# kubeflow/Code-Intelligence

Hardware: NVIDIA H100
Metric: issues/sec to 2400-d @ seq_len 512 batch 256 (higher is better)
Workload: dtype bf16

## Files before the change

code_intelligence_b200/csrc/api.cu:

```cuda
#include <algorithm>
#include <cmath>
#include <cstdarg>
#include <cstdio>
#include <cstdlib>
#include <cstring>
#include <mutex>
#include <string>
#include <vector>

#include <cuda_fp16.h>

#include "../../include/issue_emb_b200.h"
#include "kernels.h"

namespace {

thread_local std::string g_last_error;

int fail(int code, const char* fmt, ...) {
  char buf[512];
  va_list ap;
  va_start(ap, fmt);
  vsnprintf(buf, sizeof(buf), fmt, ap);
  va_end(ap);
// ... 358 lines not shown
    CK(ie::launch_tokens_time_major(ids_dev, B, T, b_pad, c.vocab_sz, c.pad_idx, h->tok.as<int>(), h->err.as<int>(), s));
    h->launches++;
  }
  if (h->use_persistent) check_persistent(h, s);
  const bool persistent = h->use_persistent != 0;
  const size_t carry_layer = static_cast<size_t>(h->max_batch) * h->y_ld;
  CK(cudaMemsetAsync(h->hcarry.p, 0, static_cast<size_t>(c.n_layers) * carry_layer * sizeof(__nv_bfloat16), s));
  const size_t slot_bytes = static_cast<size_t>(b_pad) * h->y_ld * sizeof(__nv_bfloat16);

  for (long long t0 = 0; t0 < T; t0 += chunk_T) {
    const int Tc = static_cast<int>(std::min<long long>(chunk_T, T - t0));
    const long long crow = static_cast<long long>(Tc) * b_pad;
    if (!proj) {
      CK(ie::launch_embed_gather(ids_dev, B, T, b_pad, h->emb.as<__nv_bfloat16>(), c.vocab_sz, ring_mul * h->e_pad,
                                 h->x0.as<__nv_bfloat16>(), ring_mul * h->e_pad, c.pad_idx, h->err.as<int>(),
                                 static_cast<int>(t0), Tc, s));
      h->launches++;
    }
    if ((rc = mark(h, 1, s)) != IE_OK) return rc;
    int cur = 0;
    const __nv_bfloat16* layer_in = h->x0.as<__nv_bfloat16>();
    const __nv_bfloat16* prev_ring = nullptr;
    long long layer_in_ld = ring_mul * h->e_pad;
    for (int l = 0; l < c.n_layers; ++l) {
      const bool last = (l == c.n_layers - 1);
      Layer& L = h->layers[l];
      const bool from_table = proj && l == 0;
      const bool fused = persistent && last && l > 0 && h->segs == 1 && h->fuse_last && L.w_cat.p != nullptr;
      __nv_bfloat16* ybuf = h->y[cur].as<__nv_bfloat16>();
      __nv_bfloat16* carry = h->hcarry.as<__nv_bfloat16>() + static_cast<size_t>(l) * carry_layer;
      float* cstate = h->c.as<float>() + static_cast<size_t>(l) * h->max_batch * mop;
      CUtensorMap tm_h, tm_w;
      CK(ie::make_tmap_bf16_2d(&tm_h, ybuf, static_cast<uint64_t>(ring_mul) * L.kh_pad, static_cast<uint64_t>(crow + b_pad),
                               h->y_ld, 64, 128));
      if (fused)
        CK(ie::make_tmap_bf16_2d(&tm_w, L.w_cat.p, static_cast<uint64_t>(L.kin_pad + L.kh_pad), 4ull * L.out_pad,
                                 static_cast<uint64_t>(L.kin_pad + L.kh_pad), 64, 256));
      else
        CK(ie::make_tmap_bf16_2d(&tm_w, L.w_hh.p, static_cast<uint64_t>(ring_mul) * L.kh_pad, 4ull * L.out_pad,
                                 static_cast<uint64_t>(ring_mul) * L.kh_pad, 64, 256));
      CUtensorMap tm_h64 = tm_h;
      CUtensorMap tm_x = tm_h;
      if (fused)
        CK(ie::make_tmap_bf16_2d(&tm_x, prev_ring, static_cast<uint64_t>(L.kin_pad), static_cast<uint64_t>(crow + b_pad),
                                 h->y_ld, 64, 128));
      if (h->use_mc)
        CK(ie::make_tmap_bf16_2d(&tm_h64, ybuf, static_cast<uint64_t>(ring_mul) * L.kh_pad,
                                 static_cast<uint64_t>(crow + b_pad), h->y_ld, 64, 64));
      CK(cudaMemcpyAsync(ybuf, carry, slot_bytes, cudaMemcpyDeviceToDevice, s));
      if (!from_table && !fused) {
        ie::GemmArgs g{};
        fill_gemm(h, L, g);
        g.a = layer_in;
        g.lda = layer_in_ld;
        g.d = h->gx.p;
        g.m_pad = static_cast<int>(crow);
        g.m_store = static_cast<int>(crow);
        g.diag = h->diag.as<long long>() + 8 * l + 4;
        CK(ie::launch_gemm_bf16(g, s));
        h->launches++;
      }
      if ((rc = mark(h, 2 + 2 * l, s)) != IE_OK) return rc;

      if (persistent) CK(cudaMemsetAsync(h->step_done.p, 0, static_cast<size_t>(Tc) * ng * sizeof(unsigned), s));
      ie::LstmLayerArgs q{};
      q.tm_h = tm_h; q.tm_w = tm_w; q.tm_h64 = tm_h64; q.mc = h->use_mc; q.mc_ctas = h->mc_ctas;
      q.tm_x = tm_x; q.pre_nkb = fused ? L.kin_pad / 64 : 0; q.bias = L.bias.as<float>();
      q.gx = from_table ? h->proj.p : h->gx.p;
      q.tok = from_table ? h->tok.as<int>() : nullptr;
      q.c = cstate; q.y = ybuf;
      q.raw = (l == raw_layer && raw_out != nullptr) ? h->raw.as<float>() : nullptr;
      q.pool_sum = (last && pooled) ? h->pool_sum.as<float>() : nullptr;
      q.pool_max = h->pool_max.as<float>(); q.pool_last = h->pool_last.as<float>();
      q.lengths = h->lengths.as<int>();
      q.step_done = h->step_done.as<unsigned>();
      q.abort_flag = h->err.as<unsigned>() + 1; q.spin_limit = h->spin_limit;
      q.T = Tc; q.t0 = static_cast<int>(t0); q.T_total = T; q.ng = ng;
      q.u = L.u; q.n_cta = L.n_cta; q.out_pad = L.out_pad; q.kh_pad = L.kh_pad;
      q.ldy = h->y_ld; q.raw_ld = L.out_pad;
      q.gate_mode = h->gate_mode; q.gx_bf16 = h->gx_bf16; q.segs = h->segs;
      q.num_sms = h->num_sms; q.check_only = 0; q.cooperative = h->cooperative; q.fault = h->fault;
      q.diag = h->diag.as<long long>() + 8 * l;
      q.trace = nullptr;
      if (persistent) {
        if (l == h->trace_layer && t0 == 0) {
          const int ctas = ie::lstm_layer_ctas(q);
          const long long items = (static_cast<long long>(Tc) * ng * L.n_cta + ctas - 1) / ctas;
          CK(h->trace.reserve(static_cast<size_t>(ctas) * items * 12 * sizeof(long long), true));
          q.trace = h->trace.as<long long>();
          q.trace_items = static_cast<int>(items);
          h->trace_T = static_cast<int>(items);
          h->trace_ctas = ctas;
        }
        cudaError_t e = ie::launch_lstm_layer(q, s);
        if (e == cudaErrorCooperativeLaunchTooLarge) {
          cudaGetLastError();
          return fail(IE_ERR_STATE, "the persistent recurrent kernel cannot be co-resident on this device "
                                   "(cooperative launch refused); set IE_SEQ=0 for the per-timestep fallback");
        }
        CK(e);
// ... 826 lines not shown
```

code_intelligence_b200/csrc/gemm.cu:

```cuda
#include "gemm_kernel.cuh"

namespace ie {


cudaError_t launch_gemm_bf16(const GemmArgs& g, cudaStream_t stream) {
  if (g.m_pad % kBlockM || g.k_pad % kBlockK || g.bn % 16 || g.bn < 16 || g.bn > 256 || g.n_pad % g.bn ||
      g.n_store % 16 || g.ldd % 2)
    return cudaErrorInvalidValue;
  CUtensorMap tmA, tmB;
  const int segs = g.segs == 3 ? 3 : 1;
  const uint64_t k_inner = static_cast<uint64_t>(segs == 3 ? 2 : 1) * g.k_pad;
  const long long spin_limit = g.spin_limit > 0 ? g.spin_limit : kSpinLimitDefault;
  cudaError_t e = make_tmap_bf16_2d(&tmA, g.a, k_inner, g.m_pad, g.lda, kBlockK, kBlockM);
  if (e != cudaSuccess) return e;
  e = make_tmap_bf16_2d(&tmB, g.b, k_inner, g.n_pad, g.ldb, kBlockK, kBlockN);
  if (e != cudaSuccess) return e;

  const size_t smem = 1024 + static_cast<size_t>(kGemmStages) * kGemmStageBytes + 2 * kGemmStages * 8 + 32;
  const int num_m_blocks = g.m_pad / kBlockM;
  const int num_n_blocks = (g.n_pad + kBlockN - 1) / kBlockN;
  const int num_k_blocks = g.k_pad / kBlockK;
  const int num_tiles = num_m_blocks * num_n_blocks;
  const int sms = g.num_sms > 0 ? g.num_sms : 132;
  const int grid = num_tiles < sms ? num_tiles : sms;
  const int panel = 16;

#define IE_LAUNCH(OUT, ACT, FRAG)                                                                                  \
  do {                                                                                                             \
    auto kfn = gemm_bf16_kernel<OUT, ACT, FRAG>;                                                                       \
    e = cudaFuncSetAttribute(kfn, cudaFuncAttributeMaxDynamicSharedMemorySize, static_cast<int>(smem));            \
    if (e != cudaSuccess) return e;                                                                                \
    kfn<<<grid, kGemmThreads, smem, stream>>>(tmA, tmB, reinterpret_cast<OUT*>(g.d), g.bias, g.m_store, g.n_store, \
                                              g.ldd, num_m_blocks, num_n_blocks, num_k_blocks, panel, segs,        \
                                              g.k_pad, g.abort_flag, spin_limit, g.diag, DenseEpi{});              \
  } while (0)

  if (g.frag) {
    if (g.act != 0 || g.out_bf16 == 1 || g.bias == nullptr || g.n_store % kBlockN || g.n_store != g.n_pad ||
        (g.ldd * (g.out_bf16 == 2 ? 2 : 4)) % 16)
      return cudaErrorInvalidValue;
    if (g.out_bf16 == 2) IE_LAUNCH(__half, 0, true);
    else IE_LAUNCH(float, 0, true);
  } else if (g.out_bf16 == 2) {
    if (g.act != 0) return cudaErrorInvalidValue;
    IE_LAUNCH(__half, 0, false);
  } else if (g.out_bf16) {
    if (g.act == 0) IE_LAUNCH(__nv_bfloat16, 0, false);
    else if (g.act == 1) IE_LAUNCH(__nv_bfloat16, 1, false);
    else IE_LAUNCH(__nv_bfloat16, 2, false);
  } else {
    if (g.act == 0) IE_LAUNCH(float, 0, false);
// ... 9 lines not shown
```

code_intelligence_b200/csrc/gemm_kernel.cuh:

```cuda
#pragma once
#include <cuda_fp16.h>
#include <type_traits>

#include "kernels.h"
#include "ptx.cuh"

namespace ie {

struct DenseEpi {
  static constexpr bool kSliced = false;
  static constexpr uint64_t kHintA = kEvictNormal;
  static constexpr uint64_t kHintB = kEvictLast;
  struct State {};
};

namespace {

__device__ __forceinline__ uint32_t pack_f16x2(float lo, float hi) {
  const __half2 v = __floats2half2_rn(lo, hi);
  return *reinterpret_cast<const uint32_t*>(&v);
}

constexpr int kBlockM = 128;
constexpr int kBlockN = 256;
constexpr int kBlockK = 64;
constexpr int kGemmThreads = 384;
constexpr int kGemmStages = 4;
constexpr uint32_t kABytes = kBlockM * kBlockK * 2;
constexpr uint32_t kBBytes = kBlockN * kBlockK * 2;
constexpr uint32_t kGemmStageBytes = kABytes + kBBytes;

template <typename OutT, int ACT, bool FRAG, typename Epi = DenseEpi>
__global__ void __launch_bounds__(kGemmThreads, 1)
gemm_bf16_kernel(const __grid_constant__ CUtensorMap tmA, const __grid_constant__ CUtensorMap tmB, OutT* __restrict__ D,
                 const float* __restrict__ bias, int m_store, int n_store, long long ldd, int num_m_blocks,
                 int num_n_blocks, int num_k_blocks, int panel, int segs, int k_pad, unsigned* abort_flag,
                 long long spin_limit, long long* diag, const __grid_constant__ Epi epi) {
  extern __shared__ uint8_t smem_raw[];
  const uint32_t raw = smem_u32(smem_raw);
  uint8_t* smem = smem_raw + ((1024u - (raw & 1023u)) & 1023u);

  uint64_t* full_bar = reinterpret_cast<uint64_t*>(smem + kGemmStages * kGemmStageBytes);
  uint64_t* empty_bar = full_bar + kGemmStages;
  uint32_t* abort_s = reinterpret_cast<uint32_t*>(empty_bar + kGemmStages);
  const Abort ab{abort_s, abort_flag, spin_limit};
  const int nkt = num_k_blocks * segs;

  const int warp = threadIdx.x >> 5;
  const int lane = threadIdx.x & 31;

  if (warp == 0 && lane == 0) {
    tma_prefetch_desc(&tmA);
    tma_prefetch_desc(&tmB);
    if (diag != nullptr && blockIdx.x == 0) {
      unsigned long long g;
      asm volatile("mov.u64 %0, %%globaltimer;" : "=l"(g));
      diag[0] = clock64();
      diag[1] = static_cast<long long>(g);
    }
  }
  if (warp == 1 && lane == 0) {
    for (int s = 0; s < kGemmStages; ++s) {
      mbar_init(&full_bar[s], 1);
// ... 32 lines not shown
      uint32_t phase = 0;
      for (int tile = first_tile; tile < num_tiles && !aborted(ab); tile = next_tile(tile)) {
        int m_blk, n_blk;
        decode(tile, m_blk, n_blk);
        for (int kb = 0; kb < nkt; ++kb) {
          const int seg = kb / num_k_blocks, r = kb - seg * num_k_blocks;
          mbar_wait(&empty_bar[stage], phase ^ 1, ab);
          uint8_t* sa = smem + static_cast<size_t>(stage) * kGemmStageBytes;
          mbar_arrive_expect_tx(&full_bar[stage], kGemmStageBytes);
          tma_load_2d(sa, &tmA, &full_bar[stage], (seg == 1 ? k_pad : 0) + r * kBlockK, m_blk * kBlockM, Epi::kHintA);
          tma_load_2d(sa + kABytes, &tmB, &full_bar[stage], (seg == 2 ? k_pad : 0) + r * kBlockK, n_blk * kBlockN,
                      Epi::kHintB);
          if (++stage == kGemmStages) { stage = 0; phase ^= 1; }
        }
      }
    }
  } else {
    const int wg = (warp - 4) >> 2;
    const int q = lane & 3;
    const int rbase = wg * 64 + (warp & 3) * 16 + (lane >> 2);
    const uint32_t smem_base = smem_u32(smem);
    const bool signal = (threadIdx.x & 127) == 0;
    int stage = 0;
    uint32_t phase = 0;
    float d[128];
    typename Epi::State st{};
    for (int tile = first_tile; tile < num_tiles; tile = next_tile(tile)) {
      int m_blk, n_blk;
      decode(tile, m_blk, n_blk);
      int prev = -1;
      for (int kb = 0; kb < nkt; ++kb) {
        mbar_wait(&full_bar[stage], phase, ab);
        const uint32_t sa = smem_base + stage * kGemmStageBytes;
        const uint64_t da = wgmma_desc_sw128(sa + wg * (kABytes / 2));
        const uint64_t db = wgmma_desc_sw128(sa + kABytes);
        wgmma_fence();
#pragma unroll
        for (int k = 0; k < kBlockK / 16; ++k) wgmma_m64n256k16(d, da + 2 * k, db + 2 * k, (kb | k) != 0);
        wgmma_commit();
        if (prev >= 0) {
          wgmma_wait<1>();
          if (signal) mbar_arrive(&empty_bar[prev]);
        }
        prev = stage;
        if (++stage == kGemmStages) { stage = 0; phase ^= 1; }
      }
      wgmma_wait<0>();
      wgmma_fence_regs(d);
      if (signal && prev >= 0) mbar_arrive(&empty_bar[prev]);
      if constexpr (Epi::kSliced) {
        epi.tile(d, m_blk, n_blk, wg * 64 + (warp & 3) * 16, lane, st);
        continue;
      }
      if constexpr (FRAG) {
        constexpr int kPer = 16 / static_cast<int>(sizeof(OutT));
        const float4* bq = reinterpret_cast<const float4*>(bias) + n_blk * (kBlockN / 4) + q;
        OutT* drow[2];
#pragma unroll
        for (int hr = 0; hr < 2; ++hr)
          drow[hr] = D + static_cast<long long>(m_blk * kBlockM + rbase + 8 * hr) * ldd + n_blk * kBlockN + q * kPer;
#pragma unroll
        for (int k = 0; k < 64 / kPer; ++k) {
          float4 b[kPer / 4];
#pragma unroll
          for (int i = 0; i < kPer / 4; ++i) b[i] = __ldg(bq + 4 * (k * (kPer / 4) + i));
#pragma unroll
          for (int hr = 0; hr < 2; ++hr) {
            if (m_blk * kBlockM + rbase + 8 * hr >= m_store) continue;
// ... 64 lines not shown
```

code_intelligence_b200/csrc/kernels.h:

```cpp
#pragma once
#include <cuda.h>
#include <cuda_bf16.h>
#include <cuda_runtime.h>
#include <stddef.h>
#include <stdint.h>

namespace ie {

cudaError_t make_tmap_bf16_2d(CUtensorMap* out, const void* base, uint64_t inner, uint64_t rows, uint64_t ld,
                              uint32_t box_inner, uint32_t box_rows);

__host__ __device__ inline int frag_index(int c, int elem_bytes) {
  const int q = (c & 7) >> 1;
  const int ix = 4 * (c >> 4) + 2 * ((c >> 3) & 1) + (c & 1);
  const int per_chunk = 16 / elem_bytes;
  return (ix / per_chunk * 4 + q) * per_chunk + ix % per_chunk;
}

struct GemmArgs {
  const __nv_bfloat16* a;
  const __nv_bfloat16* b;
  void* d;
  const float* bias;
  int m_pad, n_pad, k_pad;
  long long lda, ldb, ldd;
  int m_store, n_store;
  int bn;
  int act;
  int out_bf16;
  int num_sms;
  int segs;
  unsigned* abort_flag;
  long long spin_limit;
  long long* diag;
  int frag;
};
cudaError_t launch_gemm_bf16(const GemmArgs& g, cudaStream_t stream);

constexpr int kMaxBatches = 12;
struct LstmLayerArgs {
// ... 80 lines not shown
```

code_intelligence_b200/csrc/knn.cu:

```cuda
#include <algorithm>

#include "gemm_kernel.cuh"

namespace ie {

namespace {

__device__ __forceinline__ uint32_t order_key(float s) {
  const uint32_t b = __float_as_uint(s);
  return (b & 0x80000000u) ? ~b : (b | 0x80000000u);
}
__device__ __forceinline__ float key_score(uint32_t k) {
  return __uint_as_float((k & 0x80000000u) ? (k & 0x7fffffffu) : ~k);
}

__device__ __noinline__ float knn_compact(uint2* buf, int count, int kp, int lane) {
  __syncwarp();
  uint32_t t = 0;
  for (int bit = 31; bit >= 0; --bit) {
    const uint32_t c = t | (1u << bit);
    int m = 0;
    for (int i = lane; i < count; i += 32) m += buf[i].x >= c;
    if (static_cast<int>(__reduce_add_sync(~0u, static_cast<unsigned>(m))) >= kp) t = c;
  }
// ... 376 lines not shown

void knn_plan(int nq, long long n, int kp, int num_sms, int* S, int* nbs) {
  const int m_blocks = (nq + 127) / 128;
  const long long n_blocks = (n + 255) / 256;
  long long s = std::max(1, num_sms / m_blocks);
  s = std::min<long long>(s, n_blocks);
  s = std::min<long long>(s, kKnnMergeMax / kp);
  *nbs = static_cast<int>((n_blocks + s - 1) / s);
  *S = static_cast<int>((n_blocks + *nbs - 1) / *nbs);
}

cudaError_t launch_knn_stage1(const KnnStage1Args& a, cudaStream_t stream) {
  if (a.m_pad % 128 || a.k_pad % 64 || a.nq > a.m_pad) return cudaErrorInvalidValue;
  CUtensorMap tmA, tmB;
  cudaError_t e = make_tmap_bf16_2d(&tmA, a.qs, 2ull * a.k_pad, a.m_pad, 2ull * a.k_pad, kBlockK, kBlockM);
  if (e != cudaSuccess) return e;
  e = make_tmap_bf16_2d(&tmB, a.xs, 2ull * a.k_pad, static_cast<uint64_t>(a.n), 2ull * a.k_pad, kBlockK, kBlockN);
  if (e != cudaSuccess) return e;
  KnnEpi epi{};
  epi.cand = a.cand;
  epi.cnt = a.cnt;
  epi.col = a.col;
  epi.rowt = a.rowt;
  epi.nq = a.nq;
  epi.n = static_cast<int>(a.n);
  epi.S = a.S;
  epi.nbs = a.nbs;
  epi.kp = a.kp;
  epi.cosine = a.cosine;
  epi.m_blocks = a.m_pad / kBlockM;
  epi.items = epi.m_blocks * a.S;
  const int num_n_blocks = static_cast<int>((a.n + kBlockN - 1) / kBlockN);
  const int grid = std::min(epi.items, a.num_sms > 0 ? a.num_sms : 132);
  const size_t smem = 1024 + static_cast<size_t>(kGemmStages) * kGemmStageBytes + 2 * kGemmStages * 8 + 32;
  auto kfn = gemm_bf16_kernel<float, 0, false, KnnEpi>;
  e = cudaFuncSetAttribute(kfn, cudaFuncAttributeMaxDynamicSharedMemorySize, static_cast<int>(smem));
  if (e != cudaSuccess) return e;
  kfn<<<grid, kGemmThreads, smem, stream>>>(tmA, tmB, nullptr, nullptr, 0, 0, 0, epi.m_blocks, num_n_blocks,
                                            a.k_pad / kBlockK, 16, 3, a.k_pad, nullptr, kSpinLimitDefault, nullptr, epi);
  return cudaGetLastError();
}

cudaError_t launch_knn_merge_rerank(const uint2* cand, const int* cnt, int rows, int S, int kp, const float* Q,
                                    const float* X, int D, int cosine, int k, float* out_dist, int64_t* out_idx,
                                    float* dbg_score, int64_t* dbg_idx, cudaStream_t stream) {
  int P = 1;
  while (P < S * kp) P <<= 1;
  const size_t smem = static_cast<size_t>(P) * 8 + static_cast<size_t>(kp) * 16;
  auto kfn = knn_merge_rerank_kernel;
  cudaError_t e = cudaFuncSetAttribute(kfn, cudaFuncAttributeMaxDynamicSharedMemorySize, static_cast<int>(smem));
  if (e != cudaSuccess) return e;
  kfn<<<rows, 512, smem, stream>>>(cand, cnt, S, kp, P, Q, X, D, cosine, k, out_dist, out_idx, dbg_score, dbg_idx);
  return cudaGetLastError();
}

}
```

code_intelligence_b200/csrc/lstm_layer.cu:

```cuda
#include <cmath>

#include <cuda_fp16.h>

#include "kernels.h"
#include "lstm_common.cuh"
#include "ptx.cuh"

namespace ie {

namespace {

constexpr int kLThreads = 384;
constexpr int kLStages = 4;
constexpr int kLTileN = 256;
constexpr int kLRows = 128;
constexpr uint32_t kHBytes = kLRows * 64 * 2;
constexpr uint32_t kWBytes = kLTileN * 64 * 2;
constexpr uint32_t kStageBytes = kHBytes + kWBytes;

__device__ __forceinline__ void st_release_cta(uint32_t* p, uint32_t v) {
  asm volatile("st.release.cta.shared::cta.u32 [%0], %1;" ::"r"(smem_u32(p)), "r"(v) : "memory");
}
__device__ __forceinline__ uint32_t ld_acquire_cta(const uint32_t* p) {
  uint32_t v;
  asm volatile("ld.acquire.cta.shared::cta.u32 %0, [%1];" : "=r"(v) : "r"(smem_u32(p)) : "memory");
  return v;
}
__device__ __forceinline__ void wait_seq_ge(const uint32_t* p, uint32_t target, const Abort& ab) {
  if (ld_acquire_cta(p) >= target) return;
  if (aborted(ab)) return;
  const long long t0 = clock64();
  uint32_t spins = 0;
  while (ld_acquire_cta(p) < target) {
    __nanosleep(64);
    if (((++spins) & 0x3Fu) == 0 && abort_poll(ab, t0)) return;
  }
}

struct KArgs {
  const void* gx;
  const int* tok;
  const float* bias;
  float* cstate;
  __nv_bfloat16* y;
  float* raw;
  float* pool_sum;
  float* pool_max;
  float* pool_last;
  const int* lengths;
  unsigned* step_done;
  unsigned* abort_flag;
  long long spin_limit;
  long long ldy, raw_ld;
  long long* trace;
  long long* diag;
  int T, t_begin, t0, T_total, ng, tiles, out_pad, nkb, segs, kh_pad, gate_mode, trace_items, fault;
  int pre_nkb;
};

template <bool TOK, bool GXBF, bool POOL, bool MC, bool FUSE>
__device__ __forceinline__ void lstm_layer_body(const CUtensorMap& tm_h, const CUtensorMap& tm_w,
                                                const CUtensorMap& tm_h64, const CUtensorMap& tm_x, const KArgs& a) {
  extern __shared__ uint8_t smem_raw[];
  const uint32_t rawaddr = smem_u32(smem_raw);
  uint8_t* smem = smem_raw + ((1024u - (rawaddr & 1023u)) & 1023u);

  uint8_t* ring = smem;
  uint64_t* full = reinterpret_cast<uint64_t*>(ring + kLStages * kStageBytes);
  uint64_t* empty = full + kLStages;
  uint32_t* cready = reinterpret_cast<uint32_t*>(empty + kLStages);
  uint32_t* abort_s = cready + 1;
  const Abort ab{abort_s, a.abort_flag, a.spin_limit};

  const int warp = threadIdx.x >> 5;
  const int lane = threadIdx.x & 31;
  long long* const trace = a.trace;
#define IE_TRACE(slot, kk) do { if (trace && (kk) < a.trace_items) { unsigned long long _g; \
    asm volatile("mov.u64 %0, %%globaltimer;" : "=l"(_g)); \
    trace[(static_cast<long long>(blockIdx.x) * a.trace_items + (kk)) * 12 + (slot)] = static_cast<long long>(_g); } } while (0)
  const uint32_t crank = MC ? cluster_ctarank() : 0u;
  const int P = static_cast<int>(gridDim.x);
  const int tiles = a.tiles, ng = a.ng;
  const int per_batch = 2 * tiles;
  const int C = ng * per_batch;
  const long long total = static_cast<long long>(a.T) * C;
  const int b_pad = 256 * ng;
  const int nkt = a.nkb * a.segs;
  const int pre = FUSE ? a.pre_nkb : 0;
  auto decode = [&](long long n, int& t, int& g, int& half, int& j) {
    const long long s = n / C;
    const int c = static_cast<int>(n - s * C);
    t = a.t_begin + static_cast<int>(s);
    g = c / per_batch;
    const int r = c - g * per_batch;
    half = r / tiles;
    j = r - half * tiles;
  };

  if (warp == 0 && lane == 0) {
    tma_prefetch_desc(&tm_h);
    tma_prefetch_desc(&tm_w);
    if (MC) tma_prefetch_desc(&tm_h64);
    if (FUSE) tma_prefetch_desc(&tm_x);
    if (a.diag != nullptr && blockIdx.x == 0) {
      unsigned long long g;
      asm volatile("mov.u64 %0, %%globaltimer;" : "=l"(g));
      a.diag[0] = clock64();
      a.diag[1] = static_cast<long long>(g);
    }
  }
  if (warp == 1 && lane == 0) {
    for (int s = 0; s < kLStages; ++s) {
      mbar_init(&full[s], 2);
      mbar_init(&empty[s], MC ? 4 : 2);
    }
    *cready = 0;
    *abort_s = 0;
    fence_barrier_init();
  }
  if (MC) cluster_sync();
  else __syncthreads();

  if (warp < 4) {
    if (warp == 0 && lane == 0) {
      int stage = 0;
      uint32_t phase = 0;
      int k = 0;
      for (long long n = blockIdx.x; n < total && !aborted(ab); n += P, ++k) {
        int t, g, half, j;
        decode(n, t, g, half, j);
        const int row0 = t * b_pad + g * 256 + half * kLRows;
        if constexpr (FUSE) {
          for (int kb = 0; kb < pre; ++kb) {
            mbar_wait(&empty[stage], phase ^ 1, ab);
            mbar_arrive_expect_tx(&full[stage], kHBytes);
            tma_load_2d(ring + stage * kStageBytes, &tm_x, &full[stage], kb * 64, row0 + b_pad, kEvictNormal);
            if (++stage == kLStages) { stage = 0; phase ^= 1; }
          }
        }
        wait_seq_ge(cready, static_cast<uint32_t>(k + 1), ab);
        if (t > a.t_begin) fence_proxy_async();
        IE_TRACE(0, k);
        for (int kb = 0; kb < nkt; ++kb) {
          mbar_wait(&empty[stage], phase ^ 1, ab);
          mbar_arrive_expect_tx(&full[stage], kHBytes);
          const int seg = kb / a.nkb, r = kb - seg * a.nkb;
          const int kc = (seg == 1 ? a.kh_pad : 0) + r * 64;
          if constexpr (MC) {
            tma_load_2d_mc(ring + stage * kStageBytes + crank * (kHBytes / 2), &tm_h64, &full[stage], kc,
                           row0 + static_cast<int>(crank) * (kLRows / 2), static_cast<uint16_t>(0x3), kEvictNormal);
          } else {
            tma_load_2d(ring + stage * kStageBytes, &tm_h, &full[stage], kc, row0, kEvictNormal);
          }
          if (++stage == kLStages) { stage = 0; phase ^= 1; }
        }
        IE_TRACE(1, k);
      }
    } else if (warp == 1 && lane == 0) {
      int stage = 0;
      uint32_t phase = 0;
      for (long long n = blockIdx.x; n < total && !aborted(ab); n += P) {
        int t, g, half, j;
        decode(n, t, g, half, j);
        for (int kb = 0; kb < pre + nkt; ++kb) {
          mbar_wait(&empty[stage], phase ^ 1, ab);
          mbar_arrive_expect_tx(&full[stage], kWBytes);
          const int seg = FUSE ? 0 : kb / a.nkb, r = kb - seg * a.nkb;
          tma_load_2d(ring + stage * kStageBytes + kHBytes, &tm_w, &full[stage], (seg == 2 ? a.kh_pad : 0) + r * 64,
                      j * kLTileN, kEvictLast);
          if (++stage == kLStages) { stage = 0; phase ^= 1; }
        }
      }
    } else if (warp == 2 && lane == 0) {
      int k = 0;
      for (long long n = blockIdx.x; n < total && !aborted(ab); n += P, ++k) {
        int t, g, half, j;
        decode(n, t, g, half, j);
        if (t > a.t_begin)
          wait_flag_ge_relaxed(a.step_done + (t - a.t_begin - 1) * ng + g, static_cast<unsigned>(per_batch), ab);
        st_release_cta(cready, static_cast<uint32_t>(k + 1));
      }
    }
  } else {
    const int wg = (warp - 4) >> 2;
    const int q = lane & 3;
    const int rbase = wg * 64 + (warp & 3) * 16 + (lane >> 2);
    const long long lo_off = a.segs > 1 ? a.kh_pad : 0;
    const uint32_t ring_base = smem_u32(ring);
    const bool signal = (threadIdx.x & 127) == 0;
    int stage = 0;
    uint32_t phase = 0;
    int k = 0;
    float d[128];
    for (long long n = blockIdx.x; n < total; n += P, ++k) {
      int t, g, half, j;
      decode(n, t, g, half, j);
      const int tg = a.t0 + t;
      int prev = -1;
      for (int kb = 0; kb < pre + nkt; ++kb) {
        mbar_wait(&full[stage], phase, ab);
        if (kb == pre && signal && wg == 0) IE_TRACE(2, k);
        const uint32_t sa = ring_base + stage * kStageBytes;
        const uint64_t da = wgmma_desc_sw128(sa + wg * (kHBytes / 2));
        const uint64_t db = wgmma_desc_sw128(sa + kHBytes);
        wgmma_fence();
#pragma unroll
        for (int kk = 0; kk < 4; ++kk) wgmma_m64n256k16(d, da + 2 * kk, db + 2 * kk, (kb | kk) != 0);
        wgmma_commit();
        if (prev >= 0) {
          wgmma_wait<1>();
          if (signal) {
            mbar_arrive(&empty[prev]);
            if (MC) mbar_arrive_remote(&empty[prev], crank ^ 1u);
          }
        }
        prev = stage;
        if (++stage == kLStages) { stage = 0; phase ^= 1; }
      }
      wgmma_wait<0>();
      wgmma_fence_regs(d);
      if (signal && prev >= 0) {
        mbar_arrive(&empty[prev]);
        if (MC) mbar_arrive_remote(&empty[prev], crank ^ 1u);
      }
      if (signal && wg == 0) IE_TRACE(3, k);
      if (lane == 0) wait_seq_ge(cready, static_cast<uint32_t>(k + 1), ab);
      __syncwarp();
#pragma unroll
      for (int hr = 0; hr < 2; ++hr) {
        const int brow = g * 256 + half * kLRows + rbase + 8 * hr;
        const int len = POOL ? a.lengths[brow] : 1;
        const long long grow = TOK ? static_cast<long long>(__ldg(a.tok + static_cast<long long>(tg) * b_pad + brow))
                                   : static_cast<long long>(t) * b_pad + brow;
        const int unit0 = j * 64 + 4 * q;
        float* cp = a.cstate + static_cast<long long>(brow) * a.out_pad + unit0;
        __nv_bfloat16* yrow = a.y + (static_cast<long long>(t + 1) * b_pad + brow) * a.ldy + unit0;
        const long long po = static_cast<long long>(brow) * a.out_pad + unit0;
        const long long gtile = grow * (4ll * a.out_pad) + j * kLTileN;
        const float* btile = FUSE ? a.bias + j * kLTileN : nullptr;
        if constexpr (FUSE) asm volatile("" : "+l"(btile));
// ... 8 lines not shown
          const float4 cprev = (tg == 0) ? make_float4(0.0f, 0.0f, 0.0f, 0.0f)
                                         : __ldcg(reinterpret_cast<const float4*>(cp + 16 * s));
          const float cp4[4] = {cprev.x, cprev.y, cprev.z, cprev.w};
          float cn[4], hn[4];
#pragma unroll
          for (int e = 0; e < 4; ++e) {
            const int m = 4 * s + e;
            float4 gx;
            if constexpr (FUSE) {
              gx = __ldg(reinterpret_cast<const float4*>(btile) + q + 4 * m);
            } else if constexpr (GXBF) {
              const uint32_t w0 = (e & 1) ? gh[e >> 1].z : gh[e >> 1].x, w1 = (e & 1) ? gh[e >> 1].w : gh[e >> 1].y;
              const float2 f01 = __half22float2(*reinterpret_cast<const __half2*>(&w0));
              const float2 f23 = __half22float2(*reinterpret_cast<const __half2*>(&w1));
              gx = make_float4(f01.x, f01.y, f23.x, f23.y);
            } else {
              gx = __ldcs(reinterpret_cast<const float4*>(reinterpret_cast<const float*>(a.gx) + gtile) + q + 4 * m);
            }
            const float zi = d[8 * m + 2 * hr] + gx.x;
            const float zf = d[8 * m + 2 * hr + 1] + gx.y;
            const float zg = d[8 * m + 4 + 2 * hr] + gx.z;
            const float zo = d[8 * m + 4 + 2 * hr + 1] + gx.w;
            lstm_cell1(zi, zf, zg, zo, cp4[e], cn[e], hn[e], a.gate_mode);
          }
          const float4 h4 = make_float4(hn[0], hn[1], hn[2], hn[3]);
          __stcg(reinterpret_cast<float4*>(cp + 16 * s), make_float4(cn[0], cn[1], cn[2], cn[3]));
          store_h4(yrow + 16 * s, h4, lo_off);
          if (a.raw != nullptr)
            *reinterpret_cast<float4*>(a.raw + (static_cast<long long>(brow) * a.T_total + tg) * a.raw_ld + unit0 + 16 * s) = h4;
          if constexpr (POOL) pool_accumulate4(a.pool_sum, a.pool_max, a.pool_last, po + 16 * s, h4, tg, len);
        }
      }
      named_bar_sync(1, 256);
      if (threadIdx.x == 128) {
        __threadfence();
        if (a.step_done != nullptr && !(a.fault && n == C))
          red_relaxed_add(a.step_done + (t - a.t_begin) * ng + g, 1u);
        IE_TRACE(6, k);
      }
    }
  }

  __syncwarp();
  if (MC) cluster_sync();
  if (a.diag != nullptr && threadIdx.x == 0 && blockIdx.x == 0) {
    unsigned long long g;
    asm volatile("mov.u64 %0, %%globaltimer;" : "=l"(g));
    a.diag[2] = clock64();
    a.diag[3] = static_cast<long long>(g);
  }
#undef IE_TRACE
}

thread_local int g_last_max_ctas = 0;

template <bool TOK, bool GXBF, bool POOL>
__global__ void __launch_bounds__(kLThreads, 1)
lstm_layer_kernel(const __grid_constant__ CUtensorMap tm_h, const __grid_constant__ CUtensorMap tm_w,
                  const __grid_constant__ CUtensorMap tm_h64, const __grid_constant__ CUtensorMap tm_x,
                  const __grid_constant__ KArgs a) {
  lstm_layer_body<TOK, GXBF, POOL, false, false>(tm_h, tm_w, tm_h64, tm_x, a);
}

template <bool POOL>
__global__ void __launch_bounds__(kLThreads, 1)
lstm_layer_fused_kernel(const __grid_constant__ CUtensorMap tm_h, const __grid_constant__ CUtensorMap tm_w,
                        const __grid_constant__ CUtensorMap tm_h64, const __grid_constant__ CUtensorMap tm_x,
                        const __grid_constant__ KArgs a) {
  lstm_layer_body<false, true, POOL, false, true>(tm_h, tm_w, tm_h64, tm_x, a);
}

template <bool TOK>
// ... 14 lines not shown
  else kfn = lstm_layer_kernel<TOK, GXBF, POOL>;
  const size_t smem = layer_smem_bytes();
  cudaError_t e = cudaFuncSetAttribute(kfn, cudaFuncAttributeMaxDynamicSharedMemorySize, static_cast<int>(smem));
  if (e != cudaSuccess) return e;
  if (a.check_only) {
    int max_ctas = 0;
    if (MC) {
      cudaLaunchConfig_t cfg{};
      cfg.gridDim = dim3(2 * (a.num_sms / 2));
      cfg.blockDim = dim3(kLThreads);
      cfg.dynamicSmemBytes = smem;
      cfg.stream = stream;
      int clusters = 0;
      e = cudaOccupancyMaxActiveClusters(&clusters, kfn, &cfg);
      max_ctas = 2 * clusters;
    } else {
      int per_sm = 0;
      e = cudaOccupancyMaxActiveBlocksPerMultiprocessor(&per_sm, kfn, kLThreads, smem);
      max_ctas = per_sm * a.num_sms;
    }
    if (e != cudaSuccess) return e;
    g_last_max_ctas = max_ctas;
    if (MC) return max_ctas >= 2 ? cudaSuccess : cudaErrorCooperativeLaunchTooLarge;
    return max_ctas >= a.num_sms ? cudaSuccess : cudaErrorCooperativeLaunchTooLarge;
  }
  KArgs k{};
  k.gx = a.gx; k.tok = a.tok; k.bias = a.bias; k.pre_nkb = FUSE ? a.pre_nkb : 0; k.cstate = a.c; k.y = a.y; k.raw = a.raw;
  k.pool_sum = a.pool_sum; k.pool_max = a.pool_max; k.pool_last = a.pool_last; k.lengths = a.lengths;
  k.step_done = a.single_step ? nullptr : a.step_done; k.abort_flag = a.abort_flag;
  k.spin_limit = a.spin_limit > 0 ? a.spin_limit : kSpinLimitDefault;
  k.ldy = a.ldy; k.raw_ld = a.raw_ld; k.trace = a.trace; k.diag = a.diag;
  k.T = a.single_step ? 1 : a.T; k.t_begin = a.single_step ? a.t_step : 0;
  k.t0 = a.t0; k.T_total = a.T_total; k.ng = a.ng; k.tiles = tiles; k.out_pad = a.out_pad;
  k.nkb = a.kh_pad / 64; k.segs = a.segs; k.kh_pad = a.kh_pad; k.gate_mode = a.gate_mode;
  k.trace_items = a.trace_items; k.fault = a.fault;
  cudaLaunchConfig_t cfg{};
  cfg.gridDim = dim3(ctas);
  cfg.blockDim = dim3(kLThreads);
  cfg.dynamicSmemBytes = smem;
  cfg.stream = stream;
  cudaLaunchAttribute attr[1];
  int na = 0;
  if (a.cooperative && !a.single_step) {
    attr[na].id = cudaLaunchAttributeCooperative;
    attr[na].val.cooperative = 1;
    ++na;
  }
  cfg.attrs = attr;
  cfg.numAttrs = na;
  return cudaLaunchKernelEx(&cfg, kfn, a.tm_h, a.tm_w, a.tm_h64, FUSE ? a.tm_x : a.tm_h, k);
}

bool lstm_layer_mc_ok(const LstmLayerArgs& a) {
  return a.mc != 0 && !a.single_step && a.gx_bf16 && a.pool_sum == nullptr && a.pre_nkb == 0 && a.segs == 1 &&
         (a.n_cta / 2) % 2 == 0 && a.mc_ctas >= 2;
}

}

int lstm_layer_max_ctas() { return g_last_max_ctas; }

int lstm_layer_ctas(const LstmLayerArgs& a) {
  const long long per_step = static_cast<long long>(a.ng) * a.n_cta;
  if (a.single_step) return static_cast<int>(per_step);
  const long long total = a.T * per_step;
  long long ctas = lstm_layer_mc_ok(a) ? a.mc_ctas : a.num_sms;
  if (ctas > total) ctas = total;
// ... 30 lines not shown
```

code_intelligence_b200/csrc/misc.cu:

```cuda
#include <cstring>

#include "kernels.h"
#include "lstm_common.cuh"
#include "ptx.cuh"

namespace ie {

typedef CUresult (*EncodeTiledFn)(CUtensorMap*, CUtensorMapDataType, cuuint32_t, void*, const cuuint64_t*,
                                  const cuuint64_t*, const cuuint32_t*, const cuuint32_t*, CUtensorMapInterleave,
                                  CUtensorMapSwizzle, CUtensorMapL2promotion, CUtensorMapFloatOOBfill);

static EncodeTiledFn get_encode_fn() {
  static EncodeTiledFn fn = nullptr;
  if (fn == nullptr) {
    void* p = nullptr;
    cudaDriverEntryPointQueryResult q;
    if (cudaGetDriverEntryPoint("cuTensorMapEncodeTiled", &p, cudaEnableDefault, &q) == cudaSuccess &&
        q == cudaDriverEntryPointSuccess)
      fn = reinterpret_cast<EncodeTiledFn>(p);
  }
  return fn;
}

cudaError_t make_tmap_bf16_2d(CUtensorMap* out, const void* base, uint64_t inner, uint64_t rows, uint64_t ld,
                              uint32_t box_inner, uint32_t box_rows) {
  EncodeTiledFn fn = get_encode_fn();
  if (fn == nullptr) return cudaErrorNotSupported;
  if (box_inner != 64 || box_rows == 0 || box_rows > 256 || (ld * 2) % 16 != 0 ||
      (reinterpret_cast<uintptr_t>(base) & 15) != 0)
    return cudaErrorInvalidValue;
  cuuint64_t dims[2] = {inner, rows};
  cuuint64_t strides[1] = {ld * 2};
  cuuint32_t box[2] = {box_inner, box_rows};
  cuuint32_t estr[2] = {1, 1};
  CUresult r = fn(out, CU_TENSOR_MAP_DATA_TYPE_BFLOAT16, 2, const_cast<void*>(base), dims, strides, box, estr,
                  CU_TENSOR_MAP_INTERLEAVE_NONE, CU_TENSOR_MAP_SWIZZLE_128B, CU_TENSOR_MAP_L2_PROMOTION_L2_256B,
                  CU_TENSOR_MAP_FLOAT_OOB_FILL_NONE);
  return r == CUDA_SUCCESS ? cudaSuccess : cudaErrorInvalidValue;
}

namespace {

__global__ void embed_gather_kernel(const int64_t* __restrict__ ids, int B, int T, int b_pad,
                                    const uint4* __restrict__ emb, int vocab, int chunks ,
                                    uint4* __restrict__ x0, long long ldx_chunks, int pad_idx, int* err_flag, int t0, int Tc) {
  const int warps_per_block = blockDim.x >> 5;
  const long long row = static_cast<long long>(blockIdx.x) * warps_per_block + (threadIdx.x >> 5);
  const long long total = static_cast<long long>(Tc) * b_pad;
  if (row >= total) return;
  const int lane = threadIdx.x & 31;
  const int tl = static_cast<int>(row / b_pad);
  const int b = static_cast<int>(row - static_cast<long long>(tl) * b_pad);
  const int t = t0 + tl;
  long long id = pad_idx;
  if (b < B) id = ids[static_cast<long long>(b) * T + t];
  if (id < 0 || id >= vocab) {
    if (lane == 0) atomicExch(err_flag, 1);
    id = 0;
  }
  const uint4* src = emb + id * chunks;
  uint4* dst = x0 + row * ldx_chunks;
  for (int i = lane; i < chunks; i += 32) dst[i] = __ldg(src + i);
}

__global__ void tokens_time_major_kernel(const int64_t* __restrict__ ids, int B, int T, int b_pad, int vocab, int pad_idx,
                                         int* __restrict__ tok, int* err_flag) {
  const long long i = static_cast<long long>(blockIdx.x) * blockDim.x + threadIdx.x;
  const long long total = static_cast<long long>(T) * b_pad;
  if (i >= total) return;
// ... 140 lines not shown
```

code_intelligence_b200/csrc/ptx.cuh:

```cuda
#pragma once
#include <cuda.h>
#include <cuda_bf16.h>
#include <cuda_runtime.h>
#include <stdint.h>

namespace ie {

constexpr uint64_t kEvictNormal = 0x1000000000000000ull;
constexpr uint64_t kEvictFirst  = 0x12F0000000000000ull;
constexpr uint64_t kEvictLast   = 0x14F0000000000000ull;

__device__ __forceinline__ uint32_t smem_u32(const void* p) {
  return static_cast<uint32_t>(__cvta_generic_to_shared(p));
}

__device__ __forceinline__ void mbar_init(uint64_t* bar, uint32_t count) {
  asm volatile("mbarrier.init.shared::cta.b64 [%0], %1;" ::"r"(smem_u32(bar)), "r"(count) : "memory");
}
__device__ __forceinline__ void fence_barrier_init() {
  asm volatile("fence.mbarrier_init.release.cluster;" ::: "memory");
}
__device__ __forceinline__ void fence_proxy_async() { asm volatile("fence.proxy.async;" ::: "memory"); }

__device__ __forceinline__ void mbar_arrive(uint64_t* bar) {
// ... 72 lines not shown
  asm volatile(
      "cp.async.bulk.tensor.2d.shared::cluster.global.mbarrier::complete_tx::bytes.L2::cache_hint"
      " [%0], [%1, {%3, %4}], [%2], %5;"
      ::"r"(smem_u32(smem_dst)), "l"(m), "r"(smem_u32(bar)), "r"(c0), "r"(c1), "l"(hint)
      : "memory");
}

__device__ __forceinline__ void tma_load_2d_mc(void* smem_dst, const CUtensorMap* m, uint64_t* bar, int32_t c0,
                                               int32_t c1, uint16_t mask, uint64_t hint) {
  asm volatile(
      "cp.async.bulk.tensor.2d.shared::cluster.global.mbarrier::complete_tx::bytes.multicast::cluster.L2::cache_hint"
      " [%0], [%1, {%4, %5}], [%2], %3, %6;"
      ::"r"(smem_u32(smem_dst)), "l"(m), "r"(smem_u32(bar)), "h"(mask), "r"(c0), "r"(c1), "l"(hint)
      : "memory");
}

__device__ __forceinline__ uint32_t cluster_ctarank() {
  uint32_t r;
  asm volatile("mov.u32 %0, %%cluster_ctarank;" : "=r"(r));
  return r;
}
__device__ __forceinline__ void cluster_sync() {
  asm volatile("barrier.cluster.arrive.release.aligned;" ::: "memory");
  asm volatile("barrier.cluster.wait.acquire.aligned;" ::: "memory");
}

__device__ __forceinline__ uint64_t wgmma_desc_sw128(uint32_t smem_addr) {
  uint64_t d = 0;
  d |= static_cast<uint64_t>((smem_addr & 0x3FFFFu) >> 4);
  d |= 1ull << 16;
  d |= static_cast<uint64_t>(1024u >> 4) << 32;
  d |= 1ull << 62;
  return d;
}
__device__ __forceinline__ void wgmma_fence() { asm volatile("wgmma.fence.sync.aligned;" ::: "memory"); }
__device__ __forceinline__ void wgmma_commit() { asm volatile("wgmma.commit_group.sync.aligned;" ::: "memory"); }
template <int N> __device__ __forceinline__ void wgmma_wait() {
  asm volatile("wgmma.wait_group.sync.aligned %0;" ::"n"(N) : "memory");
}
__device__ __forceinline__ void wgmma_fence_regs(float (&d)[128]) {
#pragma unroll
  for (int i = 0; i < 128; ++i) asm volatile("" : "+f"(d[i])::"memory");
}

__device__ __forceinline__ void wgmma_m64n256k16(float (&d)[128], uint64_t desc_a, uint64_t desc_b, uint32_t accumulate) {
  asm volatile(
      "{\n\t"
      ".reg .pred p;\n\t"
      "setp.ne.b32 p, %130, 0;\n\t"
      "wgmma.mma_async.sync.aligned.m64n256k16.f32.bf16.bf16 {"
      "%0, %1, %2, %3, %4, %5, %6, %7, %8, %9, %10, %11, %12, %13, %14, %15, "
      "%16, %17, %18, %19, %20, %21, %22, %23, %24, %25, %26, %27, %28, %29, %30, %31, "
      "%32, %33, %34, %35, %36, %37, %38, %39, %40, %41, %42, %43, %44, %45, %46, %47, "
      "%48, %49, %50, %51, %52, %53, %54, %55, %56, %57, %58, %59, %60, %61, %62, %63, "
      "%64, %65, %66, %67, %68, %69, %70, %71, %72, %73, %74, %75, %76, %77, %78, %79, "
      "%80, %81, %82, %83, %84, %85, %86, %87, %88, %89, %90, %91, %92, %93, %94, %95, "
      "%96, %97, %98, %99, %100, %101, %102, %103, %104, %105, %106, %107, %108, %109, %110, %111, "
      "%112, %113, %114, %115, %116, %117, %118, %119, %120, %121, %122, %123, %124, %125, %126, %127}, "
      "%128, %129, p, 1, 1, 0, 0;\n\t"
      "}\n"
      : "+f"(d[0]), "+f"(d[1]), "+f"(d[2]), "+f"(d[3]), "+f"(d[4]), "+f"(d[5]), "+f"(d[6]), "+f"(d[7]),
        "+f"(d[8]), "+f"(d[9]), "+f"(d[10]), "+f"(d[11]), "+f"(d[12]), "+f"(d[13]), "+f"(d[14]), "+f"(d[15]),
        "+f"(d[16]), "+f"(d[17]), "+f"(d[18]), "+f"(d[19]), "+f"(d[20]), "+f"(d[21]), "+f"(d[22]), "+f"(d[23]),
        "+f"(d[24]), "+f"(d[25]), "+f"(d[26]), "+f"(d[27]), "+f"(d[28]), "+f"(d[29]), "+f"(d[30]), "+f"(d[31]),
        "+f"(d[32]), "+f"(d[33]), "+f"(d[34]), "+f"(d[35]), "+f"(d[36]), "+f"(d[37]), "+f"(d[38]), "+f"(d[39]),
        "+f"(d[40]), "+f"(d[41]), "+f"(d[42]), "+f"(d[43]), "+f"(d[44]), "+f"(d[45]), "+f"(d[46]), "+f"(d[47]),
// ... 52 lines not shown
```

Baseline: 3994.

## Offload step-done signaling to a producer warp and parametrize the K-block width

Thread 128 no longer runs the __threadfence and global atomic that publish per-step completion. It now writes a CTA-local 'stored' counter, and an otherwise idle producer warp (warp 3) waits on that counter and does the fence plus atomic increment of step_done. The goal is to take the global fence off the consumer warpgroups' critical path. The cost is an extra intra-CTA hop that may add latency to the cross-CTA recurrence signal. The K-block width and ring depth also become a compile-time option (32 or 64, using 64B or 128B swizzle), but the default stays 64 with 4 stages.

```diff
diff --git a/code_intelligence_b200/csrc/api.cu b/code_intelligence_b200/csrc/api.cu
--- a/code_intelligence_b200/csrc/api.cu
+++ b/code_intelligence_b200/csrc/api.cu
@@ -414,21 +414,21 @@
       float* cstate = h->c.as<float>() + static_cast<size_t>(l) * h->max_batch * mop;
       CUtensorMap tm_h, tm_w;
       CK(ie::make_tmap_bf16_2d(&tm_h, ybuf, static_cast<uint64_t>(ring_mul) * L.kh_pad, static_cast<uint64_t>(crow + b_pad),
-                               h->y_ld, 64, 128));
+                               h->y_ld, ie::kKBlock, 128));
       if (fused)
         CK(ie::make_tmap_bf16_2d(&tm_w, L.w_cat.p, static_cast<uint64_t>(L.kin_pad + L.kh_pad), 4ull * L.out_pad,
-                                 static_cast<uint64_t>(L.kin_pad + L.kh_pad), 64, 256));
+                                 static_cast<uint64_t>(L.kin_pad + L.kh_pad), ie::kKBlock, 256));
       else
         CK(ie::make_tmap_bf16_2d(&tm_w, L.w_hh.p, static_cast<uint64_t>(ring_mul) * L.kh_pad, 4ull * L.out_pad,
-                                 static_cast<uint64_t>(ring_mul) * L.kh_pad, 64, 256));
+                                 static_cast<uint64_t>(ring_mul) * L.kh_pad, ie::kKBlock, 256));
       CUtensorMap tm_h64 = tm_h;
       CUtensorMap tm_x = tm_h;
       if (fused)
         CK(ie::make_tmap_bf16_2d(&tm_x, prev_ring, static_cast<uint64_t>(L.kin_pad), static_cast<uint64_t>(crow + b_pad),
-                                 h->y_ld, 64, 128));
+                                 h->y_ld, ie::kKBlock, 128));
       if (h->use_mc)
         CK(ie::make_tmap_bf16_2d(&tm_h64, ybuf, static_cast<uint64_t>(ring_mul) * L.kh_pad,
-                                 static_cast<uint64_t>(crow + b_pad), h->y_ld, 64, 64));
+                                 static_cast<uint64_t>(crow + b_pad), h->y_ld, ie::kKBlock, 64));
       CK(cudaMemcpyAsync(ybuf, carry, slot_bytes, cudaMemcpyDeviceToDevice, s));
       if (!from_table && !fused) {
         ie::GemmArgs g{};
@@ -447,7 +447,7 @@
       if (persistent) CK(cudaMemsetAsync(h->step_done.p, 0, static_cast<size_t>(Tc) * ng * sizeof(unsigned), s));
       ie::LstmLayerArgs q{};
       q.tm_h = tm_h; q.tm_w = tm_w; q.tm_h64 = tm_h64; q.mc = h->use_mc; q.mc_ctas = h->mc_ctas;
-      q.tm_x = tm_x; q.pre_nkb = fused ? L.kin_pad / 64 : 0; q.bias = L.bias.as<float>();
+      q.tm_x = tm_x; q.pre_nkb = fused ? L.kin_pad / ie::kKBlock : 0; q.bias = L.bias.as<float>();
       q.gx = from_table ? h->proj.p : h->gx.p;
       q.tok = from_table ? h->tok.as<int>() : nullptr;
       q.c = cstate; q.y = ybuf;
diff --git a/code_intelligence_b200/csrc/gemm.cu b/code_intelligence_b200/csrc/gemm.cu
--- a/code_intelligence_b200/csrc/gemm.cu
+++ b/code_intelligence_b200/csrc/gemm.cu
@@ -4,7 +4,7 @@
 
 
 cudaError_t launch_gemm_bf16(const GemmArgs& g, cudaStream_t stream) {
-  if (g.m_pad % kBlockM || g.k_pad % kBlockK || g.bn % 16 || g.bn < 16 || g.bn > 256 || g.n_pad % g.bn ||
+  if (g.m_pad % kBlockM || g.k_pad % 64 || g.bn % 16 || g.bn < 16 || g.bn > 256 || g.n_pad % g.bn ||
       g.n_store % 16 || g.ldd % 2)
     return cudaErrorInvalidValue;
   CUtensorMap tmA, tmB;
@@ -16,7 +16,7 @@
   e = make_tmap_bf16_2d(&tmB, g.b, k_inner, g.n_pad, g.ldb, kBlockK, kBlockN);
   if (e != cudaSuccess) return e;
 
-  const size_t smem = 1024 + static_cast<size_t>(kGemmStages) * kGemmStageBytes + 2 * kGemmStages * 8 + 32;
+  const size_t smem = kGemmSmemBytes;
   const int num_m_blocks = g.m_pad / kBlockM;
   const int num_n_blocks = (g.n_pad + kBlockN - 1) / kBlockN;
   const int num_k_blocks = g.k_pad / kBlockK;
diff --git a/code_intelligence_b200/csrc/gemm_kernel.cuh b/code_intelligence_b200/csrc/gemm_kernel.cuh
--- a/code_intelligence_b200/csrc/gemm_kernel.cuh
+++ b/code_intelligence_b200/csrc/gemm_kernel.cuh
@@ -23,12 +23,13 @@
 
 constexpr int kBlockM = 128;
 constexpr int kBlockN = 256;
-constexpr int kBlockK = 64;
+constexpr int kBlockK = kKBlock;
 constexpr int kGemmThreads = 384;
-constexpr int kGemmStages = 4;
+constexpr int kGemmStages = kRingStages;
 constexpr uint32_t kABytes = kBlockM * kBlockK * 2;
 constexpr uint32_t kBBytes = kBlockN * kBlockK * 2;
 constexpr uint32_t kGemmStageBytes = kABytes + kBBytes;
+constexpr size_t kGemmSmemBytes = 1024 + static_cast<size_t>(kGemmStages) * kGemmStageBytes + 2 * kGemmStages * 8 + 32;
 
 template <typename OutT, int ACT, bool FRAG, typename Epi = DenseEpi>
 __global__ void __launch_bounds__(kGemmThreads, 1)
@@ -127,8 +128,8 @@
       for (int kb = 0; kb < nkt; ++kb) {
         mbar_wait(&full_bar[stage], phase, ab);
         const uint32_t sa = smem_base + stage * kGemmStageBytes;
-        const uint64_t da = wgmma_desc_sw128(sa + wg * (kABytes / 2));
-        const uint64_t db = wgmma_desc_sw128(sa + kABytes);
+        const uint64_t da = wgmma_desc<kBlockK>(sa + wg * (kABytes / 2));
+        const uint64_t db = wgmma_desc<kBlockK>(sa + kABytes);
         wgmma_fence();
 #pragma unroll
         for (int k = 0; k < kBlockK / 16; ++k) wgmma_m64n256k16(d, da + 2 * k, db + 2 * k, (kb | k) != 0);
diff --git a/code_intelligence_b200/csrc/kernels.h b/code_intelligence_b200/csrc/kernels.h
--- a/code_intelligence_b200/csrc/kernels.h
+++ b/code_intelligence_b200/csrc/kernels.h
@@ -6,6 +6,13 @@
 #include <stdint.h>
 
 namespace ie {
+
+#ifndef IE_KBLOCK
+#define IE_KBLOCK 64
+#endif
+constexpr int kKBlock = IE_KBLOCK;
+static_assert(kKBlock == 32 || kKBlock == 64, "k-block width must be 32 or 64 bf16");
+constexpr int kRingStages = 256 / kKBlock;
 
 cudaError_t make_tmap_bf16_2d(CUtensorMap* out, const void* base, uint64_t inner, uint64_t rows, uint64_t ld,
                               uint32_t box_inner, uint32_t box_rows);
diff --git a/code_intelligence_b200/csrc/knn.cu b/code_intelligence_b200/csrc/knn.cu
--- a/code_intelligence_b200/csrc/knn.cu
+++ b/code_intelligence_b200/csrc/knn.cu
@@ -432,7 +432,7 @@
   epi.items = epi.m_blocks * a.S;
   const int num_n_blocks = static_cast<int>((a.n + kBlockN - 1) / kBlockN);
   const int grid = std::min(epi.items, a.num_sms > 0 ? a.num_sms : 132);
-  const size_t smem = 1024 + static_cast<size_t>(kGemmStages) * kGemmStageBytes + 2 * kGemmStages * 8 + 32;
+  const size_t smem = kGemmSmemBytes;
   auto kfn = gemm_bf16_kernel<float, 0, false, KnnEpi>;
   e = cudaFuncSetAttribute(kfn, cudaFuncAttributeMaxDynamicSharedMemorySize, static_cast<int>(smem));
   if (e != cudaSuccess) return e;
diff --git a/code_intelligence_b200/csrc/lstm_layer.cu b/code_intelligence_b200/csrc/lstm_layer.cu
--- a/code_intelligence_b200/csrc/lstm_layer.cu
+++ b/code_intelligence_b200/csrc/lstm_layer.cu
@@ -11,11 +11,11 @@
 namespace {
 
 constexpr int kLThreads = 384;
-constexpr int kLStages = 4;
+constexpr int kLStages = kRingStages;
 constexpr int kLTileN = 256;
 constexpr int kLRows = 128;
-constexpr uint32_t kHBytes = kLRows * 64 * 2;
-constexpr uint32_t kWBytes = kLTileN * 64 * 2;
+constexpr uint32_t kHBytes = kLRows * kKBlock * 2;
+constexpr uint32_t kWBytes = kLTileN * kKBlock * 2;
 constexpr uint32_t kStageBytes = kHBytes + kWBytes;
 
 __device__ __forceinline__ void st_release_cta(uint32_t* p, uint32_t v) {
@@ -70,6 +70,7 @@
   uint64_t* empty = full + kLStages;
   uint32_t* cready = reinterpret_cast<uint32_t*>(empty + kLStages);
   uint32_t* abort_s = cready + 1;
+  uint32_t* stored = cready + 2;
   const Abort ab{abort_s, a.abort_flag, a.spin_limit};
 
   const int warp = threadIdx.x >> 5;
@@ -116,6 +117,7 @@
     }
     *cready = 0;
     *abort_s = 0;
+    *stored = 0;
     fence_barrier_init();
   }
   if (MC) cluster_sync();
@@ -134,7 +136,7 @@
           for (int kb = 0; kb < pre; ++kb) {
             mbar_wait(&empty[stage], phase ^ 1, ab);
             mbar_arrive_expect_tx(&full[stage], kHBytes);
-            tma_load_2d(ring + stage * kStageBytes, &tm_x, &full[stage], kb * 64, row0 + b_pad, kEvictNormal);
+            tma_load_2d(ring + stage * kStageBytes, &tm_x, &full[stage], kb * kKBlock, row0 + b_pad, kEvictNormal);
             if (++stage == kLStages) { stage = 0; phase ^= 1; }
           }
         }
@@ -145,7 +147,7 @@
           mbar_wait(&empty[stage], phase ^ 1, ab);
           mbar_arrive_expect_tx(&full[stage], kHBytes);
           const int seg = kb / a.nkb, r = kb - seg * a.nkb;
-          const int kc = (seg == 1 ? a.kh_pad : 0) + r * 64;
+          const int kc = (seg == 1 ? a.kh_pad : 0) + r * kKBlock;
           if constexpr (MC) {
             tma_load_2d_mc(ring + stage * kStageBytes + crank * (kHBytes / 2), &tm_h64, &full[stage], kc,
                            row0 + static_cast<int>(crank) * (kLRows / 2), static_cast<uint16_t>(0x3), kEvictNormal);
@@ -166,7 +168,7 @@
           mbar_wait(&empty[stage], phase ^ 1, ab);
           mbar_arrive_expect_tx(&full[stage], kWBytes);
           const int seg = FUSE ? 0 : kb / a.nkb, r = kb - seg * a.nkb;
-          tma_load_2d(ring + stage * kStageBytes + kHBytes, &tm_w, &full[stage], (seg == 2 ? a.kh_pad : 0) + r * 64,
+          tma_load_2d(ring + stage * kStageBytes + kHBytes, &tm_w, &full[stage], (seg == 2 ? a.kh_pad : 0) + r * kKBlock,
                       j * kLTileN, kEvictLast);
           if (++stage == kLStages) { stage = 0; phase ^= 1; }
         }
@@ -179,6 +181,17 @@
         if (t > a.t_begin)
           wait_flag_ge_relaxed(a.step_done + (t - a.t_begin - 1) * ng + g, static_cast<unsigned>(per_batch), ab);
         st_release_cta(cready, static_cast<uint32_t>(k + 1));
+      }
+    } else if (warp == 3 && lane == 0) {
+      int k = 0;
+      for (long long n = blockIdx.x; n < total && !aborted(ab); n += P, ++k) {
+        int t, g, half, j;
+        decode(n, t, g, half, j);
+        wait_seq_ge(stored, static_cast<uint32_t>(k + 1), ab);
+        __threadfence();
+        if (a.step_done != nullptr && !(a.fault && n == C))
+          red_relaxed_add(a.step_done + (t - a.t_begin) * ng + g, 1u);
+        IE_TRACE(6, k);
       }
     }
   } else {
@@ -201,11 +214,11 @@
         mbar_wait(&full[stage], phase, ab);
         if (kb == pre && signal && wg == 0) IE_TRACE(2, k);
         const uint32_t sa = ring_base + stage * kStageBytes;
-        const uint64_t da = wgmma_desc_sw128(sa + wg * (kHBytes / 2));
-        const uint64_t db = wgmma_desc_sw128(sa + kHBytes);
+        const uint64_t da = wgmma_desc<kKBlock>(sa + wg * (kHBytes / 2));
+        const uint64_t db = wgmma_desc<kKBlock>(sa + kHBytes);
         wgmma_fence();
 #pragma unroll
-        for (int kk = 0; kk < 4; ++kk) wgmma_m64n256k16(d, da + 2 * kk, db + 2 * kk, (kb | kk) != 0);
+        for (int kk = 0; kk < kKBlock / 16; ++kk) wgmma_m64n256k16(d, da + 2 * kk, db + 2 * kk, (kb | kk) != 0);
         wgmma_commit();
         if (prev >= 0) {
           wgmma_wait<1>();
@@ -280,12 +293,7 @@
         }
       }
       named_bar_sync(1, 256);
-      if (threadIdx.x == 128) {
-        __threadfence();
-        if (a.step_done != nullptr && !(a.fault && n == C))
-          red_relaxed_add(a.step_done + (t - a.t_begin) * ng + g, 1u);
-        IE_TRACE(6, k);
-      }
+      if (threadIdx.x == 128) st_release_cta(stored, static_cast<uint32_t>(k + 1));
     }
   }
 
@@ -366,7 +374,7 @@
   k.ldy = a.ldy; k.raw_ld = a.raw_ld; k.trace = a.trace; k.diag = a.diag;
   k.T = a.single_step ? 1 : a.T; k.t_begin = a.single_step ? a.t_step : 0;
   k.t0 = a.t0; k.T_total = a.T_total; k.ng = a.ng; k.tiles = tiles; k.out_pad = a.out_pad;
-  k.nkb = a.kh_pad / 64; k.segs = a.segs; k.kh_pad = a.kh_pad; k.gate_mode = a.gate_mode;
+  k.nkb = a.kh_pad / kKBlock; k.segs = a.segs; k.kh_pad = a.kh_pad; k.gate_mode = a.gate_mode;
   k.trace_items = a.trace_items; k.fault = a.fault;
   cudaLaunchConfig_t cfg{};
   cfg.gridDim = dim3(ctas);
diff --git a/code_intelligence_b200/csrc/misc.cu b/code_intelligence_b200/csrc/misc.cu
--- a/code_intelligence_b200/csrc/misc.cu
+++ b/code_intelligence_b200/csrc/misc.cu
@@ -26,15 +26,16 @@
                               uint32_t box_inner, uint32_t box_rows) {
   EncodeTiledFn fn = get_encode_fn();
   if (fn == nullptr) return cudaErrorNotSupported;
-  if (box_inner != 64 || box_rows == 0 || box_rows > 256 || (ld * 2) % 16 != 0 ||
+  if ((box_inner != 32 && box_inner != 64) || box_rows == 0 || box_rows > 256 || (ld * 2) % 16 != 0 ||
       (reinterpret_cast<uintptr_t>(base) & 15) != 0)
     return cudaErrorInvalidValue;
+  const CUtensorMapSwizzle swizzle = box_inner == 64 ? CU_TENSOR_MAP_SWIZZLE_128B : CU_TENSOR_MAP_SWIZZLE_64B;
   cuuint64_t dims[2] = {inner, rows};
   cuuint64_t strides[1] = {ld * 2};
   cuuint32_t box[2] = {box_inner, box_rows};
   cuuint32_t estr[2] = {1, 1};
   CUresult r = fn(out, CU_TENSOR_MAP_DATA_TYPE_BFLOAT16, 2, const_cast<void*>(base), dims, strides, box, estr,
-                  CU_TENSOR_MAP_INTERLEAVE_NONE, CU_TENSOR_MAP_SWIZZLE_128B, CU_TENSOR_MAP_L2_PROMOTION_L2_256B,
+                  CU_TENSOR_MAP_INTERLEAVE_NONE, swizzle, CU_TENSOR_MAP_L2_PROMOTION_L2_256B,
                   CU_TENSOR_MAP_FLOAT_OOB_FILL_NONE);
   return r == CUDA_SUCCESS ? cudaSuccess : cudaErrorInvalidValue;
 }
diff --git a/code_intelligence_b200/csrc/ptx.cuh b/code_intelligence_b200/csrc/ptx.cuh
--- a/code_intelligence_b200/csrc/ptx.cuh
+++ b/code_intelligence_b200/csrc/ptx.cuh
@@ -128,6 +128,18 @@
   d |= static_cast<uint64_t>(1024u >> 4) << 32;
   d |= 1ull << 62;
   return d;
+}
+__device__ __forceinline__ uint64_t wgmma_desc_sw64(uint32_t smem_addr) {
+  uint64_t d = 0;
+  d |= static_cast<uint64_t>((smem_addr & 0x3FFFFu) >> 4);
+  d |= 1ull << 16;
+  d |= static_cast<uint64_t>(512u >> 4) << 32;
+  d |= 2ull << 62;
+  return d;
+}
+template <int KBLOCK> __device__ __forceinline__ uint64_t wgmma_desc(uint32_t smem_addr) {
+  static_assert(KBLOCK == 32 || KBLOCK == 64, "k-block width must be 32 or 64 bf16");
+  return KBLOCK == 64 ? wgmma_desc_sw128(smem_addr) : wgmma_desc_sw64(smem_addr);
 }
 __device__ __forceinline__ void wgmma_fence() { asm volatile("wgmma.fence.sync.aligned;" ::: "memory"); }
 __device__ __forceinline__ void wgmma_commit() { asm volatile("wgmma.commit_group.sync.aligned;" ::: "memory"); }
```

After: 4112, median of 6. 1.03x the previous value.
